# daiszh/A-TVSNet

Hardware: AMD Instinct MI355X
Metric: depth-maps/sec at 640x512xD=192, N=5 views (higher is better)
Workload: dtype f32 (fp16x2 split operands); 1 GPU; 1 depth map(s) per step: 5 views (1 ref + 4 src) 640x512, D=192, example.py multi-view pipeline; voxels=3932160, parallelism=single GPU, world_size=1, rccl_ranks=0, launch=HIP graph replay, batched per-view networks, inflight=1

## Files before the change

### a-tvsnet_amd/csrc/conv_stem.hip

```cpp
#include "conv_common.h"

namespace {

constexpr int ST_TZ = 4, ST_TY = 8, ST_TX = 32;
constexpr int ST_HZ = ST_TZ + 2, ST_HY = ST_TY + 2, ST_HX = ST_TX + 2;
typedef unsigned u32x4 __attribute__((ext_vector_type(4)));
__device__ float rs_zeros[8];
constexpr int RS_PF = (ST_HZ * ST_HY * ST_HX + 255) / 256;
#ifndef RS_WAVES
#define RS_WAVES 2
#endif
constexpr int RS_GRID = RS_WAVES * 256;
constexpr int RS_STG = 64 * 9;

template <int CIN>
__global__ __launch_bounds__(256) void conv_stem_kernel(const float* __restrict__ x, const float* __restrict__ w,
                                                        const float* __restrict__ pbias, float* __restrict__ y,
                                                        double* __restrict__ stats, int D, int H, int W, int ldy, int ycoff,
                                                        int relu, int tiles_y, int tiles_x, int tiles) {
  __shared__ float tile[ST_HZ * ST_HY * ST_HX * CIN];
  __shared__ double s_red[4][2][8];
  const int tid = threadIdx.x;
  const int grp = blockIdx.x / tiles, t = blockIdx.x - grp * tiles;
  const int x0 = (t % tiles_x) * ST_TX, y0 = ((t / tiles_x) % tiles_y) * ST_TY, z0 = (t / (tiles_x * tiles_y)) * ST_TZ;
  const size_t vol = (size_t)D * H * W;
  const float* xg = x + (size_t)grp * vol * CIN;
  for (int s = tid; s < ST_HZ * ST_HY * ST_HX * CIN; s += 256) {
    const int c = s % CIN, v = s / CIN;
    const int xx = v % ST_HX, yy = (v / ST_HX) % ST_HY, zz = v / (ST_HX * ST_HY);
    const int gz = z0 + zz - 1, gy = y0 + yy - 1, gx = x0 + xx - 1;
    float val = 0.f;
    if ((unsigned)gz < (unsigned)D && (unsigned)gy < (unsigned)H && (unsigned)gx < (unsigned)W)
      val = xg[(((size_t)gz * H + gy) * W + gx) * CIN + c];
    tile[s] = val;
  }
  __syncthreads();
  const int lx = tid & 31, ly = tid >> 5;
  const int xo = x0 + lx, yo = y0 + ly;
  const bool col_ok = xo < W && yo < H;
  float acc[ST_TZ][8];
#pragma unroll
  for (int z = 0; z < ST_TZ; ++z)
#pragma unroll
    for (int k = 0; k < 8; ++k) acc[z][k] = 0.f;
#pragma unroll 1
  for (int kd = 0; kd < 3; ++kd)
#pragma unroll 1
    for (int j = 0; j < 9; ++j) {
      const float* wk = w + ((kd * 9 + j) * CIN) * 8;
      float wr[CIN][8];
#pragma unroll
      for (int c = 0; c < CIN; ++c)
#pragma unroll
// ... 222 lines not shown
        const bool ok = yy < H && xx < W && zo < D;
        const u32x4 bits = {__builtin_bit_cast(unsigned, v.x), __builtin_bit_cast(unsigned, v.y),
                            __builtin_bit_cast(unsigned, v.z), __builtin_bit_cast(unsigned, v.w)};
        const unsigned off = ok ? (unsigned)(((z * H + yy) * W + xx) * 8 + hf * 4) * 4u : ybytes;
        __builtin_amdgcn_raw_buffer_store_b128(bits, c == 0 ? yrsrc : (c == 1 ? yrsrc1 : yrsrc2), off, 0, ATVS_BUF_NT);
      }
    } else
#pragma unroll
    for (int i = 0; i < 8; ++i) {
      const int r = i >> 2, xi = (i & 3) * 8 + (lane >> 3), c = lane & 7;
      const float4 v = stg[(r * 32 + xi) * 9 + c];
      const int yy = y0 + 2 * wave + r, xx = x0 + xi;
      const bool ok = yy < H && xx < W && zo < D;
      const u32x4 bits = {__builtin_bit_cast(unsigned, v.x), __builtin_bit_cast(unsigned, v.y),
                          __builtin_bit_cast(unsigned, v.z), __builtin_bit_cast(unsigned, v.w)};
      __builtin_amdgcn_raw_buffer_store_b128(bits, yrsrc, ok ? (unsigned)(((z * H + yy) * W + xx) * 32 + c * 4) * 4u : ybytes, 0, ATVS_BUF_NT);
    }
    __builtin_amdgcn_fence(__ATOMIC_RELEASE, "wavefront");
    __builtin_amdgcn_wave_barrier();
    __builtin_amdgcn_fence(__ATOMIC_ACQUIRE, "wavefront");
  }
  if (stats) {
    double v[48];
#pragma unroll
    for (int k = 0; k < 24; ++k) {
      v[k] = (double)ssum[k];
      v[24 + k] = (double)ssq[k];
    }
    int c0 = 0;
    rs_halve<24>(v, 1, lane, c0);
    rs_halve<12>(v, 2, lane, c0);
    rs_halve<6>(v, 4, lane, c0);
    rs_halve<3>(v, 8, lane, c0);
#pragma unroll
    for (int i = 0; i < 3; ++i) {
      v[i] += __shfl_xor(v[i], 16);
      v[i] += __shfl_xor(v[i], 32);
    }
    if (lane < 16) {
      double* row = &s_red[wave][0][0];
#pragma unroll
      for (int i = 0; i < 3; ++i) row[c0 + i] = v[i];
    }
    __syncthreads();
    if (tid < 48) {
      const int which = tid / 24, col = tid % 24;
      stats[((size_t)id * 2 + which) * 24 + col] =
          (s_red[0][which][col] + s_red[1][which][col]) + (s_red[2][which][col] + s_red[3][which][col]);
    }
  }
  }
}

}

extern "C" long atvs_conv_stem_rows(int D, int H, int W) {
  return (long)((D + ST_TZ - 1) / ST_TZ) * ((H + ST_TY - 1) / ST_TY) * ((W + ST_TX - 1) / ST_TX);
}

extern "C" int atvs_conv_stem_f32(const float* x, const float* w, const float* plane_bias, float* y, double* stats_partial,
                                  int groups, int D, int H, int W, int Cin, int ldy, int y_coff, int relu,
                                  atvs_stream_t stream) {
  if (!x || !w || !y) return ATVS_ERR_NULL;
  if (groups <= 0 || D <= 0 || H <= 0 || W <= 0 || (Cin != 1 && Cin != 2)) return ATVS_ERR_SHAPE;
  if (y_coff < 0 || y_coff + 8 > ldy || (ldy % 4) || (y_coff % 4)) return ATVS_ERR_SHAPE;
  if (plane_bias && D < 2) return ATVS_ERR_ARG;
  const int ty = (H + ST_TY - 1) / ST_TY, tx = (W + ST_TX - 1) / ST_TX;
  const long tiles = atvs_conv_stem_rows(D, H, W);
  if (tiles * groups > 0x7fffffffL) return ATVS_ERR_SHAPE;
  dim3 grid((unsigned)(tiles * groups)), block(256);
  hipStream_t s = as_stream(stream);
  if (Cin == 1)
    hipLaunchKernelGGL((conv_stem_kernel<1>), grid, block, 0, s, x, w, plane_bias, y, stats_partial, D, H, W, ldy, y_coff, relu,
                       ty, tx, (int)tiles);
  else
    hipLaunchKernelGGL((conv_stem_kernel<2>), grid, block, 0, s, x, w, plane_bias, y, stats_partial, D, H, W, ldy, y_coff, relu,
                       ty, tx, (int)tiles);
  ATVS_LAUNCH_CHECK();
  return ATVS_OK;
}

extern "C" int atvs_refine_stems_f32(const float* photo_raw, const float* geo, const float* geo_plane_bias, const float* prob,
                                     const float* hull, const float* w, float* y, double* stats_partial, int groups, int D,
                                     int H, int W, long y_planar, atvs_stream_t stream) {
  if ((!photo_raw && !y_planar) || !geo || !prob || !hull || !w || !y) return ATVS_ERR_NULL;
  if (groups <= 0 || D <= 0 || H <= 0 || W <= 0) return ATVS_ERR_SHAPE;
  if (y_planar && y_planar < (long)D * H * W * 8) return ATVS_ERR_ARG;
  if (geo_plane_bias && D < 2) return ATVS_ERR_ARG;
  if ((double)H * W * 128.0 * ST_TZ >= 4294967296.0) return ATVS_ERR_SHAPE;
  const int ty = (H + ST_TY - 1) / ST_TY, tx = (W + ST_TX - 1) / ST_TX;
  const long tiles = atvs_conv_stem_rows(D, H, W);
  if (tiles * groups > 0x7fffffffL) return ATVS_ERR_SHAPE;
  const long total = tiles * groups;
  const dim3 grid((unsigned)(total < RS_GRID ? total : RS_GRID));
  if (y_planar)
    hipLaunchKernelGGL(refine_stems_kernel<true>, grid, dim3(256), 0, as_stream(stream), photo_raw, geo, geo_plane_bias, prob,
                       hull, w, y, stats_partial, D, H, W, ty, tx, (int)tiles, groups, y_planar);
  else
    hipLaunchKernelGGL(refine_stems_kernel<false>, grid, dim3(256), 0, as_stream(stream), photo_raw, geo, geo_plane_bias, prob,
                       hull, w, y, stats_partial, D, H, W, ty, tx, (int)tiles, groups, 0L);
  ATVS_LAUNCH_CHECK();
  return ATVS_OK;
}

extern "C" int atvs_refine_stems_pack(const float* w_geo, const float* w_prob, const float* w_hull, float* packed) {
  if (!w_geo || !w_prob || !w_hull || !packed) return ATVS_ERR_NULL;
  for (int t = 0; t < 27; ++t)
    for (int k = 0; k < 8; ++k) {
      packed[(t * 4 + 0) * 8 + k] = w_geo[(t * 2 + 0) * 8 + k];
      packed[(t * 4 + 1) * 8 + k] = w_geo[(t * 2 + 1) * 8 + k];
      packed[(t * 4 + 2) * 8 + k] = w_prob[t * 8 + k];
      packed[(t * 4 + 3) * 8 + k] = w_hull[t * 8 + k];
    }
  return ATVS_OK;
}
```

### a-tvsnet_amd/ops/base.py

```python

import ctypes
import os

import torch

from .. import _lib


_ERR = {-1: 'null pointer', -2: 'bad shape', -3: 'bad argument', -4: 'launch failed'}


class Config(object):
    _DEFAULTS = dict(
        split16=os.environ.get('ATVS_SPLIT16', '1') == '1',
        split_off=frozenset(v for v in os.environ.get('ATVS_SPLIT_OFF', '').split(',') if v),
        xb=os.environ.get('ATVS_SPLIT16', '1') == '1',
        planar=True,
        pieces=os.environ.get('ATVS_PIECES', '1') == '1',
        planar_concat=os.environ.get('ATVS_PLANAR_CONCAT', '1') != '0',
        conv_c16=True, deconv_up=True, stem=True, conv2d_lds=True, conv1x1=True, xp1w=True, xpair=True, siblings=True,
        aanet_fused=os.environ.get('ATVS_AANET_FUSED', '1') != '0',
        bottleneck=os.environ.get('ATVS_BOTTLENECK', '1') != '0',
        prologue=True, sum_on_load=os.environ.get('ATVS_SUM_ON_LOAD', '1') != '0',
        norm3d=os.environ.get('ATVS_NORM3D', '1') != '0', head_sum=os.environ.get('ATVS_HEAD_SUM', '1') != '0',
        force_impl=None, fused_finalize=False,
        side_streams=os.environ.get('ATVS_SIDE_STREAMS', '1') != '0')

    def __init__(self):
        for k, v in self._DEFAULTS.items():
            object.__setattr__(self, k, v)

    def __setattr__(self, name, value):
        if name not in self._DEFAULTS:
            raise AttributeError('ops.cfg has no switch %r (known: %s)' % (name, ', '.join(sorted(self._DEFAULTS))))
        if name == 'split_off':
            value = frozenset(value)
        elif name == 'force_impl':
            if value not in (None, 'tiled', 'gather'):
                raise ValueError('force_impl: None | "tiled" | "gather"')
        else:
            value = bool(value)
        object.__setattr__(self, name, value)
        if name == 'split16':
            object.__setattr__(self, 'xb', value)

    def snapshot(self):
        return {k: getattr(self, k) for k in self._DEFAULTS}


cfg = Config()


class configure(object):

    def __init__(self, clear_pack_cache=False, **switches):
        for k in switches:
            if k not in Config._DEFAULTS:
                raise AttributeError('ops.cfg has no switch %r' % k)
        self._new, self._clear = switches, clear_pack_cache

    def __enter__(self):
        self._old = cfg.snapshot()
        for k in sorted(self._new, key=lambda n: n != 'split16'):
            setattr(cfg, k, self._new[k])
        if self._clear:
            from .packing import clear_pack_cache
            clear_pack_cache()
        return cfg

    def __exit__(self, *exc):
        for k, v in self._old.items():
            object.__setattr__(cfg, k, v)
        if self._clear:
            from .packing import clear_pack_cache
            clear_pack_cache()
        return False

# ... 123 lines not shown
```

### a-tvsnet_amd/ops/convolution.py

```python

import ctypes

import torch

from .. import _lib
from .base import _Timed, _call, _dev_ok, _new, _p, _side_stream, _stats, _stats_buffer, _stream, cfg
from .packing import (_abi_pack, _fold_cache, _virt_cache, _xkind, conv_taps, deconv_s2_class_taps, deconv_up_ok,
    pack_conv3d_b, pack_conv_c16, pack_conv_c16b, pack_conv_weights, pack_conv_weights_tiled, pack_conv_xp,
    pack_conv_xp_sibling, pack_deconv_up, planar_pieces_decode, planar_stride, planar_view, split_on)
from .geometry import tile_planes
from .norm import LAZY, PendingBN, PendingSum, _param_groups, bn_apply, channel_stats, copy_channels, siblings_prologue_ok
from .launch import (Fin, XPAIR_TAPS, _fin_counter, _from5, _to5, _xpair_virtual_kernel, conv1x1, conv2d_lds, conv_blocks,
    conv_launch, conv_plan, conv_tiled_launch, conv_xp_launch, pack_conv2d_lds, tiled_blocks, tiled_tile_y, xp_blocks)


def conv(x, key, w_host, stride=1, dilation=1, padding='SAME', explicit_pad=None, bias=None, residual=None,
         relu=False, want_stats=False, out=None, y_coff=0, plane_bias=None, groups=None, in_params=None,
         in_relu=False, in_sum=None):
    x5, nsp = _to5(x, groups, 'conv input')
    G, ins = x5.shape[0], tuple(x5.shape[1:4])
    cin, cout = int(w_host.shape[-2]), int(w_host.shape[-1])
    if cin != x5.shape[4]:
        raise ValueError('conv %s: input has %d channels, kernel wants %d' % (key, x5.shape[4], cin))
    y5 = _to5(out, groups, 'conv output buffer')[0] if out is not None else None
# ... 224 lines not shown
    cv, cc = sv.cv, sv.const.shape[-1]
    wv, planes = _fold_split_weights(key, w_host, sv.chan_map, cv, cc)
    pb = conv(sv.const, (key, 'planes'), planes, stride=stride, groups=B)
    return conv(sv.var, (key, 'var'), wv, stride=stride, want_stats=want_stats, plane_bias=pb, out=out, y_coff=y_coff,
                groups=B)


def planar_concat_ok(shape):
    D, h, w = (int(v) for v in shape)
    return (cfg.planar_concat and cfg.planar and _xkind() == 'xb' and cfg.prologue and cfg.force_impl is None
            and siblings_ok((D, h, w), 32, 8, 16) and 4.0 * 4 * planar_stride(D, h, w) < 2.0 ** 40)


def photo_pieces_ok(shape, chan):
    return cfg.pieces and chan in (16, 32, 64) and planar_concat_ok(shape)


def conv_split_into_plane(sv, key, w_host, buf, plane, planar):
    D, H, W = planar
    B, K, pstride = buf.shape
    if (sv.planar and (not sv.pieces or sv.planar != (D, H, W))) or sv.shape[0] != B or tuple(sv.shape[1:4]) != (D, H, W) or pstride != planar_stride(D, H, W) \
            or not buf.is_contiguous() or int(w_host.shape[-1]) != 8 or sv.cv % 8:
        raise ValueError('conv_split_into_plane: shapes')
    cv, cc = sv.cv, sv.const.shape[-1]
    wv, planes = _fold_split_weights(key, w_host, sv.chan_map, cv, cc)
    pb = conv(sv.const, (key, 'planes'), planes, stride=1, groups=B)
    pk = pack_conv_xp((key, 'var'), wv, buf.device)
    if pk.kind != 'xb':
        raise ValueError('conv_split_into_plane: the split-fp16 x-pair kernel only')
    blocks = xp_blocks(D, H, W, B)
    st, sbuf = _stats(buf, blocks, 16, D * H * W, B)
    if sv.pieces:
        conv_xp_launch(sv._var, pk, buf, 0, None, False, sbuf, pb, ldy=8, y_gstride=K * pstride, y_off=int(plane) * pstride,
                       planar=sv.planar, pieces=True)
    else:
        conv_xp_launch(sv.var, pk, buf, 0, None, False, sbuf, pb, ldy=8, y_gstride=K * pstride, y_off=int(plane) * pstride)
    return st


def refine_stems(photo_raw, geo_var, geo_plane_bias, prob, hull, key, w_geo, w_prob, w_hull, planar_out=None):
    import numpy as np
    B, D, H, W, _ = geo_var.shape
    if planar_out is not None and (tuple(planar_out.shape) != (B, 4, planar_stride(D, H, W)) or not planar_out.is_contiguous()):
        raise ValueError('refine_stems: planar_out must be a contiguous (B, 4, planar_stride(D,h,w)) buffer')
    photo_raw = geo_var if planar_out is not None else photo_raw
    if tuple(np.shape(w_geo)) != (3, 3, 3, 2, 8) or tuple(np.shape(w_prob)) != (3, 3, 3, 1, 8) \
            or tuple(np.shape(w_hull)) != (3, 3, 3, 1, 8):
        raise ValueError('refine_stems: kernels [3,3,3,2,8], [3,3,3,1,8], [3,3,3,1,8]')
    pk = _abi_pack('stems', key, (w_geo, w_prob, w_hull), photo_raw.device, 'refine_stems_pack', 27 * 4 * 8, cin=4, cout=24)
    buf = _new(photo_raw, (B, D, H, W, 32)) if planar_out is None else planar_out
    st, sbuf = _stats(photo_raw, _lib.lib().atvs_conv_stem_rows(D, H, W), 24, D * H * W, B)
    if _dev_ok(photo_raw, geo_var, geo_plane_bias, prob, hull, buf):
        with _Timed(key, (D, H, W, 4), 24, B):
            _call('atvs_refine_stems_f32', _p(photo_raw if planar_out is None else None), _p(geo_var), _p(geo_plane_bias),
                  _p(prob), _p(hull), _p(pk.wp), _p(buf), _p(sbuf), B, D, H, W,
                  ctypes.c_long(planar_stride(D, H, W) if planar_out is not None else 0), _stream())
    return buf, st


def siblings_ok(shape, cin, cout, cout2):
    return (cfg.xp1w and cfg.xpair and cfg.siblings and cfg.force_impl != 'gather' and len(shape) == 3 and cout == 8
            and cout2 == 16 and cin % 8 == 0 and (shape[2] >= 24 or cfg.force_impl == 'tiled'))


def conv_siblings(x, key, w_host, key2, w2_host, plane_bias=None, plane_bias2=None, groups=None, planar=False, pieces=False):
    prologue = None
    if isinstance(x, LAZY):
        if not siblings_prologue_ok(x):
            raise ValueError('conv_siblings: this lazy input must be materialised first')
        if isinstance(x, PendingBN) and x.planar and x._final is None:
            planar = x.planar
        x, prologue = x.prologue()
    if planar:
        D, H, W = planar
        if (prologue is not None and _xkind() != 'xb') or groups is None or x.dim() != 3 \
                or not x.is_contiguous() or x.shape[2] != planar_stride(D, H, W):
            raise ValueError('conv_siblings(planar=(D,H,W)): a contiguous (G, Cin/8, planar_stride) buffer (a prologue only '
                             'on the split-fp16 kernel)')
        G, K = x.shape[:2]
        x5, nsp, cin = x, 3, K * 8
    else:
        x5, nsp = _to5(x, groups, 'conv_siblings input')
        G, D, H, W, cin = x5.shape
    if nsp != 3 or not siblings_ok((D, H, W), cin, int(w_host.shape[-1]), int(w2_host.shape[-1])):
        raise ValueError('conv_siblings: unsupported shapes')
    pk = pack_conv_xp(key, w_host, x.device)
    pk2 = pack_conv_xp_sibling(key2, w2_host, x.device)
    if pk.cin != cin or pk2.cin != cin:
        raise ValueError('conv_siblings %s: input has %d channels' % (key, cin))
    D2, H2, W2 = (D + 1) // 2, (H + 1) // 2, (W + 1) // 2
    lead = () if groups is None else (G,)
    y, y2 = _new(x, lead + (D, H, W, 8)), _new(x, lead + (D2, H2, W2, 16))
    blocks = xp_blocks(D, H, W, G)
    st, sbuf = _stats(x, blocks, 16, D * H * W, G)
    st2, sbuf2 = _stats(x, blocks, 16, D2 * H2 * W2, G)
    if plane_bias is not None and tuple(plane_bias.shape) != lead + (H, W, 24):
        raise ValueError('conv_siblings %s: plane_bias %s' % (key, tuple(plane_bias.shape)))
    if plane_bias2 is not None and tuple(plane_bias2.shape) != lead + (H2, W2, 48):
        raise ValueError('conv_siblings %s: plane_bias2 %s' % (key2, tuple(plane_bias2.shape)))
    if prologue is not None and prologue[0] is not None:
        prologue = (_to5(prologue[0], groups, 'conv_siblings second source')[0],) + tuple(prologue[1:])
    if pieces and (not planar or prologue is not None or _xkind() != 'xb'):
        raise ValueError('conv_siblings(pieces=True): a chunk-planar input without a prologue, on the split-operand kernel')
    conv_xp_launch(x5, pk, y, 0, None, False, sbuf, plane_bias, sibling=(pk2, y2, 0, sbuf2, plane_bias2),
                   prologue=prologue, planar=planar, pieces=pieces)
    return (y, st), (y2, st2)

# ... 177 lines not shown
```

### include/atvsnet_hip.h

```cpp
#ifndef ATVSNET_HIP_H
#define ATVSNET_HIP_H

#include <stddef.h>
#include <stdint.h>

#ifdef __cplusplus
extern "C" {
#endif

typedef void* atvs_stream_t;

enum {
  ATVS_OK = 0,
  ATVS_ERR_NULL = -1,
  ATVS_ERR_SHAPE = -2,
  ATVS_ERR_ARG = -3,
  ATVS_ERR_LAUNCH = -4
};

#define ATVS_ABI_VERSION 50
int atvs_abi_version(void);
const char* atvs_target_arch(void);


int atvs_get_homographies(const float* left_cam, const float* right_cam, const float* depth_start,
                          const float* depth_interval, float* homographies, int depth_num,
                          int inverse_depth, atvs_stream_t stream);

int atvs_warp_planes(const float* src, const float* homographies, const float* ref,
                     const float* depth_start, const float* depth_interval, float* out, float* mask_out,
                     int D, int h, int w, int C, int ld_out, int c_off, int mode, int rep, long planar, int pieces,
                     atvs_stream_t stream);

int atvs_build_cost_volume(const float* ref_feature, const float* view_feature, const float* homographies,
                           float* cost_volume, int D, int h, int w, int C, atvs_stream_t stream);

int atvs_tile_planes(const float* src, float* out, int D, int h, int w, int C, int ld_out, int c_off,
                     atvs_stream_t stream);

int atvs_geo_ref_planes(const float* depth_ref, const float* depth_start, const float* depth_interval,
                        float* out, int D, int h, int w, int ld_out, int c_off, atvs_stream_t stream);
int atvs_geo_volume(const float* depth_ref, const float* view_depth, const float* homographies, const float* depth_start,
                    const float* depth_interval, float* out, int D, int h, int w, int ld_out, int c_off, int rep,
                    atvs_stream_t stream);

int atvs_visual_hull(const float* ref_depth, const float* view_depth_in_ref, const float* homographies,
                     const float* depth_start, const float* depth_interval, float* out, int D, int h, int w,
                     int inverse_depth, atvs_stream_t stream);

int atvs_warp_by_depth(const float* src, const float* left_cam, const float* right_cam, const float* depth,
                       float* out, float* mask_out, float* pose_ws, int h, int w, int C, int method,
                       int inverse_depth, atvs_stream_t stream);

int atvs_warp_by_depth_err(const float* src, const float* ref, const float* left_cam, const float* right_cam,
                           const float* depth, float* out, int ld_out, int c_off, int h, int w, int C, int method,
                           int inverse_depth, int copy_ref, atvs_stream_t stream);

int atvs_interpolate(const float* src, const float* x, const float* y, float* out, float* mask_out, long n,
                     int h, int w, int C, int method, atvs_stream_t stream);

int atvs_pixel_grids(float* out, int h, int w, atvs_stream_t stream);

int atvs_transform_depth(const float* depth, const float* left_cam, const float* right_cam, float* out,
                         float* ws14, int h, int w, int inverse_depth, atvs_stream_t stream);
int atvs_transform_depth_batch_supported(int h, int w);
int atvs_transform_depth_batch(const float* const* depth, const float* const* left_cam, const float* const* right_cam,
                               float* const* out, int n, int h, int w, int inverse_depth, atvs_stream_t stream);

int atvs_absdiff_mask(const float* a, const float* b, const float* mask, float* out, int npix, int C,
                      atvs_stream_t stream);


int atvs_softargmin(const float* cost, const float* depth_start, const float* depth_interval,
// ... 95 lines not shown
int atvs_conv1x1_b_pack_size(int Cin, int Cout, long* packed_bytes);
int atvs_conv1x1_b_pack(const float* w, int Cin, int Cout, unsigned char* packed);
long atvs_conv1x1_b_rows(long pixels);
int atvs_conv1x1_b_f32(const float* x, const unsigned char* packed_w, const float* bias, const float* residual,
                       const float* in_params, int in_relu, float* y, double* stats_partial, int groups, long pixels,
                       int Cin, int Cout, int ldy, int y_coff, int relu, atvs_stream_t stream);

int atvs_bottleneck_b_supported(int C, int dilation);
long atvs_bottleneck_b_rows(int C, int H, int W);
int atvs_bottleneck_b_f32(const float* x, const float* in_params, const unsigned char* w1, const float* b1,
                          const unsigned char* w2, const float* b2, const unsigned char* w3, const float* b3, float* y,
                          double* stats_partial, int G, int H, int W, int C, int dilation, atvs_stream_t stream);

int atvs_conv3d_b_supported(int Cin, int Cout);
int atvs_conv3d_b_pack_size(int Cin, int Cout, long* packed_bytes);
int atvs_conv3d_b_pack(const float* w, int Cin, int Cout, unsigned char* packed);
int atvs_conv3d_b_f32(const float* x, const unsigned char* packed_w, const float* bias, float* y, double* stats_partial,
                      int groups, int D, int H, int W, int Cin, int Cout, int ldy, int y_coff, int relu, atvs_stream_t stream);
int atvs_conv3d_b_norm_f32(const float* x, const float* in_params, int in_relu, const unsigned char* packed_w, const float* bias,
                           float* y, double* stats_partial, int groups, int D, int H, int W, int Cin, int Cout, int ldy,
                           int y_coff, int relu, atvs_stream_t stream);

int atvs_conv3d_s2b_supported(int Cin, int Cout);
long atvs_conv3d_s2b_grid(int Do, int Ho, int Wo, int groups);
int atvs_conv3d_s2b_pack_size(int Cin, int Cout, long* packed_bytes);
int atvs_conv3d_s2b_pack(const float* w, int Cin, int Cout, unsigned char* packed);
int atvs_conv3d_s2b_f32(const float* x, const unsigned char* packed_w, const float* bias, float* y, double* stats_partial,
                        int groups, int D, int H, int W, int Cin, int Cout, int ldy, int y_coff, int relu, atvs_stream_t stream);
int atvs_conv3d_s2b_norm_f32(const float* x, const float* in_params, int in_relu, const unsigned char* packed_w,
                             const float* bias, float* y, double* stats_partial, int groups, int D, int H, int W, int Cin,
                             int Cout, int ldy, int y_coff, int relu, atvs_stream_t stream);

long atvs_deconv_up_b_grid(int D, int H, int W, int Cout, int groups);
int atvs_deconv_up_b_supported(int Cin, int Cout);
int atvs_deconv_up_b_pack_size(int Cin, int Cout, long* packed_bytes);
int atvs_deconv_up_b_pack(const float* w, int Cin, int Cout, unsigned char* packed);
int atvs_deconv_up_b_f32(const float* x, const unsigned char* packed_w, float* y, double* stats_partial, int groups, int D, int H,
                         int W, int Cin, int Cout, int ldy, int y_coff, int relu, int stats_ld, int stats_coff,
                         atvs_stream_t stream);

int atvs_deconv_up_b_sum_supported(int Cin, int Cout);
int atvs_deconv_up_b_sum_f32(const float* x0, const float* params0, const float* x1, const float* params1, const float* x2,
                             const float* params2, int relu_mask, const unsigned char* packed_w, float* y, double* stats_partial,
                             int groups, int D, int H, int W, int Cin, int Cout, int ldy, int y_coff, int relu, int stats_ld,
                             int stats_coff, atvs_stream_t stream);
long atvs_conv_stem_rows(int D, int H, int W);
int atvs_conv_stem_f32(const float* x, const float* w, const float* plane_bias, float* y, double* stats_partial,
                       int groups, int D, int H, int W, int Cin, int ldy, int y_coff, int relu, atvs_stream_t stream);

int atvs_refine_stems_pack(const float* w_geo, const float* w_prob, const float* w_hull, float* packed);
int atvs_refine_stems_f32(const float* photo_raw, const float* geo, const float* geo_plane_bias, const float* prob,
                          const float* hull, const float* w, float* y, double* stats_partial, int groups, int D, int H,
                          int W, long y_planar, atvs_stream_t stream);

int atvs_conv3d_8to1(const float* x, const float* w, float* y, int groups, int D, int H, int W, atvs_stream_t stream);
int atvs_conv3d_8to1_bn2(const float* x0, const float* params0, const float* x1, const float* params1, int relu_mask,
                         const float* w, float* y, int groups, int D, int H, int W, atvs_stream_t stream);



int atvs_bn_finalize(const double* stats_partial, int groups, long num_blocks, int cpad, int fold, long count,
                     const float* beta, float eps, float* params, int C, int* nonfinite_flag, atvs_stream_t stream);

long atvs_channel_stats_num_blocks(long rows);
int atvs_channel_stats(const float* x, int groups, long rows, int C, double* stats_partial, atvs_stream_t stream);

int atvs_bn_apply(const float* x, const float* params, float* y, int groups, long rows, int C, int ld, int c_off,
                  int relu, atvs_stream_t stream);

int atvs_bn_add(const float* x0, const float* params0, const float* x1, const float* params1, const float* x2,
                const float* params2, float* y, int groups, long rows, int C, int relu_mask, atvs_stream_t stream);
int atvs_bn_add_plus(const float* x0, const float* params0, const float* x1, const float* params1, const float* x2,
                     const float* params2, float* y, const float* base, float* y2, int groups, long rows, int C, int relu_mask,
                     atvs_stream_t stream);

int atvs_add_n(const float* a, const float* b, const float* c, float* y, long n, atvs_stream_t stream);

long atvs_avg_pool_ws_floats(int H, int W, int C, int stride);
int atvs_avg_pool_same(const float* x, float* y, float* ws, int groups, int H, int W, int C, int pool, int stride,
                       atvs_stream_t stream);

int atvs_resize_bilinear(const float* x, float* y, int groups, int H, int W, int C, int Ho, int Wo, int ld_out,
                         int c_off, atvs_stream_t stream);

int atvs_copy_channels(const float* src, float* dst, long rows, int C, int ld_src, int src_off, int ld_dst,
                       int dst_off, atvs_stream_t stream);

int atvs_stack(const float* const* srcs, int n, long elems, float* dst, atvs_stream_t stream);


int atvs_aanet_combine(const float* const* sr_ptrs, const float* const* x_ptrs, int nv, float* out, long V,
                       atvs_stream_t stream);

int atvs_aanet_b_supported(int C, int nv);
int atvs_aanet_b_pack_size(long* packed_bytes);
int atvs_aanet_b_pack(const float* w_shared, const float* w_unique, unsigned char* packed);
int atvs_aanet_b_f32(const float* const* x, int nv, const unsigned char* packed_w, float* out, int D, int H, int W,
                     atvs_stream_t stream);

int atvs_aanet_partial(const float* const* sr_ptrs, const float* const* x_ptrs, int nv, int stage,
                       const float* ssum, const float* umax, float* out, long V, atvs_stream_t stream);

int atvs_divide(const float* num, const float* den, float* out, long n, atvs_stream_t stream);


int atvs_fusibile(const float* cams, const float* normals_depths, const float* images, int nviews, int ref, int rows,
// ... 80 lines not shown
```

Before: 59.90 depth-maps/sec.

## Split refine-stems kernel into producer/consumer wave roles with double-buffered halo

Adds a 512-thread persistent refine_stems kernel with specialized wavefronts. Four waves run the 27-tap FMA loop from LDS with software-pipelined weight and voxel loads. The other four waves, at raised priority, prefetch the next tile's halo into a second LDS buffer through buffer loads and handle bias, statistics and output stores. The aim is to overlap global memory latency and epilogue work with the tap arithmetic that the previous single-role kernel ran serially. In exchange it uses a large dynamic LDS footprint, one block per CU, and extra LDS barriers. An env switch, on by default, keeps the old kernel selectable.

Result: no change. 60.31 depth-maps/sec, median of 3 (+0.7%).

```diff
diff --git a/a-tvsnet_amd/csrc/conv_stem.hip b/a-tvsnet_amd/csrc/conv_stem.hip
--- a/a-tvsnet_amd/csrc/conv_stem.hip
+++ b/a-tvsnet_amd/csrc/conv_stem.hip
@@ -1,4 +1,10 @@
 #include "conv_common.h"
+
+typedef float rs_f32x2 __attribute__((ext_vector_type(2)));
+__device__ rs_f32x2 rs_buffer_load_x2(__amdgpu_buffer_rsrc_t rsrc, int voffset, int soffset, int aux)
+    __asm("llvm.amdgcn.raw.ptr.buffer.load.v2f32");
+__device__ float rs_buffer_load_x1(__amdgpu_buffer_rsrc_t rsrc, int voffset, int soffset, int aux)
+    __asm("llvm.amdgcn.raw.ptr.buffer.load.f32");
 
 namespace {
 
@@ -327,6 +333,332 @@
   }
 }
 
+constexpr int RS_IMG = ST_HZ * ST_HY * ST_HX;
+constexpr int RS2_SLOT = 4 * RS_STG;
+constexpr int RS2_LDS = (2 * RS_IMG + 2 * RS2_SLOT) * 16 + 4 * 48 * 8;
+constexpr int RS2_GRID = 256;
+
+#ifdef ATVS_RS_DEBUG
+__device__ unsigned long long atvs_dbg_rs[256 * 8 * 8];
+#define RSDBG(i) { unsigned long long t_ = clock64(); dbg_acc[i] += t_ - dbg_t; dbg_t = t_; }
+#else
+#define RSDBG(i)
+#endif
+
+struct RsTaps { int b[32]; };
+constexpr RsTaps rs_make_taps() {
+  RsTaps t{};
+  for (int i = 0; i < 27; ++i) t.b[i] = (((i / 9) * ST_HY + (i % 9) / 3) * ST_HX + i % 3) * 16;
+  return t;
+}
+__constant__ RsTaps rs_taps = rs_make_taps();
+
+__device__ __forceinline__ void rs_lds_barrier() { asm volatile("s_waitcnt lgkmcnt(0)\n\ts_barrier" ::: "memory"); }
+
+template <bool PLANAR>
+__global__ __launch_bounds__(512, 1) void refine_stems_kernel_roles(const float* __restrict__ photo, const float* __restrict__ geo,
+                                                                  const float* __restrict__ geo_pb, const float* __restrict__ prob,
+                                                                  const float* __restrict__ hull, const float* __restrict__ w,
+                                                                  float* __restrict__ y, double* __restrict__ stats, int D, int H,
+                                                                  int W, int tiles_y, int tiles_x, int tiles, int groups, long pstride) {
+  extern __shared__ __attribute__((aligned(16))) unsigned char rs_smem[];
+  float4* const img = reinterpret_cast<float4*>(rs_smem);
+  float4* const slots = img + 2 * RS_IMG;
+  double* const s_red = reinterpret_cast<double*>(slots + 2 * RS2_SLOT);
+  const int tid = threadIdx.x & 255, lane = tid & 63;
+  const int wave = __builtin_amdgcn_readfirstlane(threadIdx.x >> 6), w4 = wave & 3;
+  const size_t vol = (size_t)D * H * W;
+  const int total = tiles * groups;
+  const int n = (total - (int)blockIdx.x + (int)gridDim.x - 1) / (int)gridDim.x;
+#ifdef ATVS_RS_DEBUG
+  unsigned long long dbg_acc[8] = {0, 0, 0, 0, 0, 0, 0, 0};
+  unsigned long long dbg_t = clock64();
+#endif
+
+  if (wave < 4) {
+    typedef float f32x2 __attribute__((ext_vector_type(2)));
+    const int lx = tid & 31, ly = tid >> 5;
+    rs_lds_barrier();
+#pragma unroll 1
+    for (int i = 0; i < n; ++i) {
+      const float4* im = img + (i & 1) * RS_IMG + ly * ST_HX + lx;
+      f32x2 acc2[ST_TZ][12];
+#pragma unroll
+      for (int z = 0; z < ST_TZ; ++z)
+#pragma unroll
+        for (int k = 0; k < 12; ++k) acc2[z][k] = (f32x2){0.f, 0.f};
+      typedef const float __attribute__((address_space(4))) * rs_cptr;
+      uintptr_t wa_ = reinterpret_cast<uintptr_t>(w);
+      asm volatile("" : "+s"(wa_));
+      const rs_cptr wt = reinterpret_cast<rs_cptr>(wa_);
+      f32x4 v0[ST_TZ], v1[ST_TZ];
+      f32x2 wA[8], wB[8];
+      int ob1 = rs_taps.b[1], ob2 = rs_taps.b[2];
+      auto issue_v = [&](int tp, f32x4* vb, int ob) __attribute__((always_inline)) {
+        const f32x4* src = reinterpret_cast<const f32x4*>(reinterpret_cast<const unsigned char*>(im) + ob);
+#pragma unroll
+        for (int z = 0; z < ST_TZ; ++z) vb[z] = src[z * ST_HY * ST_HX];
+      };
+      auto issue_w = [&](int tp, int part, f32x2* wb) __attribute__((always_inline)) {
+        const rs_cptr wk = wt + tp * 32 + part * 16;
+#pragma unroll
+        for (int k = 0; k < 8; ++k) wb[k] = (f32x2){wk[2 * k], wk[2 * k + 1]};
+      };
+      auto pin = [&](f32x4* vb) __attribute__((always_inline)) {
+#pragma unroll
+        for (int z = 0; z < ST_TZ; ++z) asm volatile("" : "+v"(vb[z]));
+      };
+      auto tap = [&](int tp, f32x4* vc, f32x4* vn, int ob, bool more) __attribute__((always_inline)) {
+        pin(vc);
+#pragma unroll
+        for (int z = 0; z < ST_TZ; ++z) {
+          const f32x2 vx = {vc[z].x, vc[z].x}, vy = {vc[z].y, vc[z].y};
+#pragma unroll
+          for (int k = 0; k < 4; ++k) {
+            acc2[z][k] = __builtin_elementwise_fma(vx, wA[k], acc2[z][k]);
+            acc2[z][k] = __builtin_elementwise_fma(vy, wA[4 + k], acc2[z][k]);
+          }
+        }
+        __builtin_amdgcn_sched_barrier(0);
+        __builtin_amdgcn_s_waitcnt(0xc07f);
+        if (more) {
+          issue_w(tp + 1, 0, wA);
+          issue_v(tp + 1, vn, ob);
+        }
+        __builtin_amdgcn_sched_barrier(0);
+#pragma unroll
+        for (int z = 0; z < ST_TZ; ++z) {
+          const f32x2 vz = {vc[z].z, vc[z].z}, vw = {vc[z].w, vc[z].w};
+#pragma unroll
+          for (int k = 0; k < 4; ++k) {
+            acc2[z][4 + k] = __builtin_elementwise_fma(vz, wB[k], acc2[z][4 + k]);
+            acc2[z][8 + k] = __builtin_elementwise_fma(vw, wB[4 + k], acc2[z][8 + k]);
+          }
+        }
+        __builtin_amdgcn_sched_barrier(0);
+        __builtin_amdgcn_s_waitcnt(0xc07f);
+        if (more) issue_w(tp + 1, 1, wB);
+        __builtin_amdgcn_sched_barrier(0);
+      };
+      issue_w(0, 0, wA);
+      issue_w(0, 1, wB);
+      issue_v(0, v0, 0);
+      __builtin_amdgcn_s_waitcnt(0xc07f);
+#pragma unroll 1
+      for (int tp = 0; tp < 26; tp += 2) {
+        const int nb1 = rs_taps.b[tp + 3], nb2 = rs_taps.b[tp + 4];
+        tap(tp, v0, v1, ob1, true);
+        tap(tp + 1, v1, v0, ob2, true);
+        ob1 = nb1;
+        ob2 = nb2;
+      }
+      tap(26, v0, v1, 0, false);
+      RSDBG(0)
+#pragma unroll
+      for (int z = 0; z < ST_TZ; ++z) {
+        float4* stg = slots + (z & 1) * RS2_SLOT + w4 * RS_STG;
+#pragma unroll
+        for (int k = 0; k < 12; k += 2) stg[lane * 9 + 2 + k / 2] = make_float4(acc2[z][k].x, acc2[z][k].y, acc2[z][k + 1].x, acc2[z][k + 1].y);
+        RSDBG(1)
+        rs_lds_barrier();
+        RSDBG(2)
+      }
+    }
+    rs_lds_barrier();
+#ifdef ATVS_RS_DEBUG
+    if (lane == 0) {
+      dbg_acc[7] = (unsigned long long)n;
+      for (int j = 0; j < 8; ++j) atvs_dbg_rs[(blockIdx.x * 8 + wave) * 8 + j] = dbg_acc[j];
+    }
+#endif
+    return;
+  }
+
+#ifndef ATVS_RS_PRIO
+#define ATVS_RS_PRIO 3
+#endif
+  __builtin_amdgcn_s_setprio(ATVS_RS_PRIO);
+  float4 pf[RS_PF];
+  int rel[RS_PF], hyy[RS_PF], hxx[RS_PF];
+#pragma unroll
+  for (int i = 0; i < RS_PF; ++i) {
+    const int s = tid + i * 256;
+    const int xx = s % ST_HX, yy = (s / ST_HX) % ST_HY, zz = s / (ST_HX * ST_HY);
+    rel[i] = (zz * H + yy) * W + xx;
+    hyy[i] = s < RS_IMG ? yy : -0x40000000;
+    hxx[i] = xx;
+  }
+  auto request = [&](int id) __attribute__((always_inline)) {
+    const int grp = id / tiles, t = id - grp * tiles;
+    const int x0 = (t % tiles_x) * ST_TX, y0 = ((t / tiles_x) % tiles_y) * ST_TY, z0 = (t / (tiles_x * tiles_y)) * ST_TZ;
+    const unsigned vbytes = (unsigned)vol * 4u;
+    const __amdgpu_buffer_rsrc_t grs = __builtin_amdgcn_make_buffer_rsrc(const_cast<float*>(geo) + (size_t)grp * vol * 2, 0, 2 * vbytes, 0x00020000);
+    const __amdgpu_buffer_rsrc_t prs = __builtin_amdgcn_make_buffer_rsrc(const_cast<float*>(prob) + (size_t)grp * vol, 0, vbytes, 0x00020000);
+    const __amdgpu_buffer_rsrc_t hrs = __builtin_amdgcn_make_buffer_rsrc(const_cast<float*>(hull) + (size_t)grp * vol, 0, vbytes, 0x00020000);
+    const int vb = ((z0 - 1) * H + (y0 - 1)) * W + (x0 - 1);
+    const int ylo = 1 - y0, xlo = 1 - x0;
+#pragma unroll
+    for (int i = 0; i < RS_PF; ++i) {
+      const int vx = vb + rel[i];
+      const bool ok = (unsigned)(hyy[i] - ylo) < (unsigned)H && (unsigned)(hxx[i] - xlo) < (unsigned)W && vx >= 0;
+      const int o4 = ok ? vx * 4 : 0x40000000;
+      const rs_f32x2 g2 = rs_buffer_load_x2(grs, o4 * 2, 0, 0);
+      pf[i] = make_float4(g2.x, g2.y, rs_buffer_load_x1(prs, o4, 0, 0), rs_buffer_load_x1(hrs, o4, 0, 0));
+    }
+  };
+  auto land = [&](float4* image) __attribute__((always_inline)) {
+#pragma unroll
+    for (int i = 0; i < RS_PF; ++i)
+      if (tid + i * 256 < RS_IMG) image[tid + i * 256] = pf[i];
+  };
+  auto stats_row = [&](int id) __attribute__((always_inline)) {
+    typedef unsigned u32x2 __attribute__((ext_vector_type(2)));
+    const int c = tid < 48 ? tid : 47;
+    const double s4 = (s_red[c] + s_red[48 + c]) + (s_red[96 + c] + s_red[144 + c]);
+    const __amdgpu_buffer_rsrc_t srsrc = __builtin_amdgcn_make_buffer_rsrc(stats + (size_t)id * 48, 0, 384, 0x00020000);
+    __builtin_amdgcn_raw_buffer_store_b64(__builtin_bit_cast(u32x2, s4), srsrc, tid < 48 ? (unsigned)tid * 8u : 384u, 0, 0);
+  };
+  request(blockIdx.x);
+  land(img);
+  request(n > 1 ? blockIdx.x + gridDim.x : blockIdx.x);
+  rs_lds_barrier();
+  const int lx = tid & 31, ly = tid >> 5;
+#pragma unroll 1
+  for (int i = 0; i < n; ++i) {
+    const int id = blockIdx.x + i * gridDim.x;
+    const int grp = id / tiles, t = id - grp * tiles;
+    const int x0 = (t % tiles_x) * ST_TX, y0 = ((t / tiles_x) % tiles_y) * ST_TY, z0 = (t / (tiles_x * tiles_y)) * ST_TZ;
+    land(img + ((i + 1) & 1) * RS_IMG);
+    RSDBG(0)
+    request(blockIdx.x + (i + 2 < n ? i + 2 : n - 1) * gridDim.x);
+    float* yg = PLANAR ? y + (size_t)grp * 4 * pstride + pstride : y + (size_t)grp * vol * 32;
+    const unsigned ybytes = (unsigned)((size_t)H * W * (PLANAR ? 32 : 128) * ST_TZ);
+    const __amdgpu_buffer_rsrc_t yrsrc = __builtin_amdgcn_make_buffer_rsrc(yg + (size_t)z0 * H * W * (PLANAR ? 8 : 32), 0, ybytes, 0x00020000);
+    const __amdgpu_buffer_rsrc_t yrsrc1 = __builtin_amdgcn_make_buffer_rsrc(yg + (PLANAR ? pstride : 0) + (size_t)z0 * H * W * 8, 0, ybytes, 0x00020000);
+    const __amdgpu_buffer_rsrc_t yrsrc2 = __builtin_amdgcn_make_buffer_rsrc(yg + (PLANAR ? 2 * pstride : 0) + (size_t)z0 * H * W * 8, 0, ybytes, 0x00020000);
+    const int xo = x0 + lx, yo = y0 + ly;
+    const bool col_ok = xo < W && yo < H;
+    const float* pbg = geo_pb ? geo_pb + (size_t)grp * H * W * 24 : nullptr;
+    float4 bb[ST_TZ][2];
+#pragma unroll
+    for (int z = 0; z < ST_TZ; ++z) {
+      const bool ok = col_ok && z0 + z < D;
+      const float* pb = ok && pbg ? pbg + ((size_t)yo * W + xo) * 24 + plane_variant(z0 + z - 1, D) * 8 : rs_zeros;
+      bb[z][0] = ld4(pb);
+      bb[z][1] = ld4(pb + 4);
+    }
+    float ssum[24], ssq[24];
+#pragma unroll
+    for (int k = 0; k < 24; ++k) ssum[k] = ssq[k] = 0.f;
+    float4 ph[ST_TZ][2];
+    if (!PLANAR) {
+      const float* phg = photo + (size_t)grp * vol * 8;
+#pragma unroll
+      for (int z = 0; z < ST_TZ; ++z) {
+        const bool ok = xo < W && yo < H && z0 + z < D;
+        const float* pp = ok ? phg + (((size_t)(z0 + z) * H + yo) * W + xo) * 8 : rs_zeros;
+        ph[z][0] = ld4(pp);
+        ph[z][1] = ld4(pp + 4);
+      }
+    }
+    RSDBG(1)
+#pragma unroll
+    for (int z = 0; z < ST_TZ; ++z) {
+      const int zo = z0 + z;
+      rs_lds_barrier();
+      RSDBG(2)
+      float4* stg = slots + (z & 1) * RS2_SLOT + w4 * RS_STG;
+      if (z == 0 && i > 0 && stats) stats_row(id - (int)gridDim.x);
+      {
+        float a24[24];
+#pragma unroll
+        for (int k = 0; k < 24; k += 4) {
+          const float4 q = stg[lane * 9 + 2 + k / 4];
+          a24[k] = q.x; a24[k + 1] = q.y; a24[k + 2] = q.z; a24[k + 3] = q.w;
+        }
+        const float4 b0 = bb[z][0], b1 = bb[z][1];
+        if (pbg) {
+          a24[0] += b0.x; a24[1] += b0.y; a24[2] += b0.z; a24[3] += b0.w;
+          a24[4] += b1.x; a24[5] += b1.y; a24[6] += b1.z; a24[7] += b1.w;
+          stg[lane * 9 + 2] = make_float4(a24[0], a24[1], a24[2], a24[3]);
+          stg[lane * 9 + 3] = make_float4(a24[4], a24[5], a24[6], a24[7]);
+        }
+        const bool ok = col_ok && zo < D;
+#pragma unroll
+        for (int k = 0; k < 24; ++k) {
+          const float a = ok ? a24[k] : 0.f;
+          ssum[k] += a;
+          ssq[k] += a * a;
+        }
+      }
+      if (!PLANAR) {
+        stg[lane * 9] = ph[z][0];
+        stg[lane * 9 + 1] = ph[z][1];
+      }
+      __builtin_amdgcn_fence(__ATOMIC_RELEASE, "wavefront");
+      __builtin_amdgcn_wave_barrier();
+      __builtin_amdgcn_fence(__ATOMIC_ACQUIRE, "wavefront");
+      if (PLANAR) {
+#pragma unroll
+        for (int j = 0; j < 6; ++j) {
+          const int c = j >> 1, r = j & 1, xi = lane >> 1, hf = lane & 1;
+          const float4 q = stg[(r * 32 + xi) * 9 + 2 + c * 2 + hf];
+          const int yy = y0 + 2 * w4 + r, xx = x0 + xi;
+          const bool ok = yy < H && xx < W && zo < D;
+          const u32x4 bits = {__builtin_bit_cast(unsigned, q.x), __builtin_bit_cast(unsigned, q.y),
+                              __builtin_bit_cast(unsigned, q.z), __builtin_bit_cast(unsigned, q.w)};
+          const unsigned off = ok ? (unsigned)(((z * H + yy) * W + xx) * 8 + hf * 4) * 4u : ybytes;
+          __builtin_amdgcn_raw_buffer_store_b128(bits, c == 0 ? yrsrc : (c == 1 ? yrsrc1 : yrsrc2), off, 0, ATVS_BUF_NT);
+        }
+      } else {
+#pragma unroll
+        for (int j = 0; j < 8; ++j) {
+          const int r = j >> 2, xi = (j & 3) * 8 + (lane >> 3), c = lane & 7;
+          const float4 q = stg[(r * 32 + xi) * 9 + c];
+          const int yy = y0 + 2 * w4 + r, xx = x0 + xi;
+          const bool ok = yy < H && xx < W && zo < D;
+          const u32x4 bits = {__builtin_bit_cast(unsigned, q.x), __builtin_bit_cast(unsigned, q.y),
+                              __builtin_bit_cast(unsigned, q.z), __builtin_bit_cast(unsigned, q.w)};
+          __builtin_amdgcn_raw_buffer_store_b128(bits, yrsrc, ok ? (unsigned)(((z * H + yy) * W + xx) * 32 + c * 4) * 4u : ybytes, 0, ATVS_BUF_NT);
+        }
+      }
+      RSDBG(3)
+    }
+    if (stats) {
+      double sv[48];
+#pragma unroll
+      for (int k = 0; k < 24; ++k) {
+        sv[k] = (double)ssum[k];
+        sv[24 + k] = (double)ssq[k];
+      }
+      int c0 = 0;
+      rs_halve<24>(sv, 1, lane, c0);
+      rs_halve<12>(sv, 2, lane, c0);
+      rs_halve<6>(sv, 4, lane, c0);
+      rs_halve<3>(sv, 8, lane, c0);
+#pragma unroll
+      for (int j = 0; j < 3; ++j) {
+        sv[j] += __shfl_xor(sv[j], 16);
+        sv[j] += __shfl_xor(sv[j], 32);
+      }
+      if (lane < 16) {
+        double* row = s_red + w4 * 48;
+#pragma unroll
+        for (int j = 0; j < 3; ++j) row[c0 + j] = sv[j];
+      }
+    }
+    RSDBG(4)
+  }
+  rs_lds_barrier();
+  if (stats) stats_row((int)blockIdx.x + (n - 1) * (int)gridDim.x);
+#ifdef ATVS_RS_DEBUG
+  if (lane == 0) {
+    dbg_acc[7] = (unsigned long long)n;
+    for (int j = 0; j < 8; ++j) atvs_dbg_rs[(blockIdx.x * 8 + wave) * 8 + j] = dbg_acc[j];
+  }
+#endif
+}
+
 }
 
 extern "C" long atvs_conv_stem_rows(int D, int H, int W) {
@@ -355,9 +687,9 @@
   return ATVS_OK;
 }
 
-extern "C" int atvs_refine_stems_f32(const float* photo_raw, const float* geo, const float* geo_plane_bias, const float* prob,
-                                     const float* hull, const float* w, float* y, double* stats_partial, int groups, int D,
-                                     int H, int W, long y_planar, atvs_stream_t stream) {
+static int refine_stems_launch(bool roles, const float* photo_raw, const float* geo, const float* geo_plane_bias, const float* prob,
+                               const float* hull, const float* w, float* y, double* stats_partial, int groups, int D, int H, int W,
+                               long y_planar, atvs_stream_t stream) {
   if ((!photo_raw && !y_planar) || !geo || !prob || !hull || !w || !y) return ATVS_ERR_NULL;
   if (groups <= 0 || D <= 0 || H <= 0 || W <= 0) return ATVS_ERR_SHAPE;
   if (y_planar && y_planar < (long)D * H * W * 8) return ATVS_ERR_ARG;
@@ -367,6 +699,21 @@
   const long tiles = atvs_conv_stem_rows(D, H, W);
   if (tiles * groups > 0x7fffffffL) return ATVS_ERR_SHAPE;
   const long total = tiles * groups;
+  if (roles && (double)D * H * W < 134217728.0) {
+    const dim3 grid((unsigned)(total < RS2_GRID ? total : RS2_GRID));
+    static AtvsAttrOnce once_planar, once_rows;
+    if (y_planar) {
+      if (const int rc_ = atvs_set_max_lds_once(once_planar, reinterpret_cast<const void*>(&refine_stems_kernel_roles<true>), RS2_LDS)) return rc_;
+      hipLaunchKernelGGL(refine_stems_kernel_roles<true>, grid, dim3(512), RS2_LDS, as_stream(stream), photo_raw, geo, geo_plane_bias,
+                         prob, hull, w, y, stats_partial, D, H, W, ty, tx, (int)tiles, groups, y_planar);
+    } else {
+      if (const int rc_ = atvs_set_max_lds_once(once_rows, reinterpret_cast<const void*>(&refine_stems_kernel_roles<false>), RS2_LDS)) return rc_;
+      hipLaunchKernelGGL(refine_stems_kernel_roles<false>, grid, dim3(512), RS2_LDS, as_stream(stream), photo_raw, geo, geo_plane_bias,
+                         prob, hull, w, y, stats_partial, D, H, W, ty, tx, (int)tiles, groups, 0L);
+    }
+    ATVS_LAUNCH_CHECK();
+    return ATVS_OK;
+  }
   const dim3 grid((unsigned)(total < RS_GRID ? total : RS_GRID));
   if (y_planar)
     hipLaunchKernelGGL(refine_stems_kernel<true>, grid, dim3(256), 0, as_stream(stream), photo_raw, geo, geo_plane_bias, prob,
@@ -378,6 +725,24 @@
   return ATVS_OK;
 }
 
+extern "C" int atvs_refine_stems_f32(const float* photo_raw, const float* geo, const float* geo_plane_bias, const float* prob,
+                                     const float* hull, const float* w, float* y, double* stats_partial, int groups, int D,
+                                     int H, int W, long y_planar, atvs_stream_t stream) {
+  return refine_stems_launch(true, photo_raw, geo, geo_plane_bias, prob, hull, w, y, stats_partial, groups, D, H, W, y_planar, stream);
+}
+
+extern "C" int atvs_refine_stems_serial_f32(const float* photo_raw, const float* geo, const float* geo_plane_bias, const float* prob,
+                                            const float* hull, const float* w, float* y, double* stats_partial, int groups, int D,
+                                            int H, int W, long y_planar, atvs_stream_t stream) {
+  return refine_stems_launch(false, photo_raw, geo, geo_plane_bias, prob, hull, w, y, stats_partial, groups, D, H, W, y_planar, stream);
+}
+
+#ifdef ATVS_RS_DEBUG
+extern "C" int atvs_debug_read_rs(void* host) {
+  return (int)hipMemcpyFromSymbol(host, HIP_SYMBOL(atvs_dbg_rs), sizeof(atvs_dbg_rs));
+}
+#endif
+
 extern "C" int atvs_refine_stems_pack(const float* w_geo, const float* w_prob, const float* w_hull, float* packed) {
   if (!w_geo || !w_prob || !w_hull || !packed) return ATVS_ERR_NULL;
   for (int t = 0; t < 27; ++t)
diff --git a/a-tvsnet_amd/ops/base.py b/a-tvsnet_amd/ops/base.py
--- a/a-tvsnet_amd/ops/base.py
+++ b/a-tvsnet_amd/ops/base.py
@@ -23,6 +23,7 @@
         bottleneck=os.environ.get('ATVS_BOTTLENECK', '1') != '0',
         prologue=True, sum_on_load=os.environ.get('ATVS_SUM_ON_LOAD', '1') != '0',
         norm3d=os.environ.get('ATVS_NORM3D', '1') != '0', head_sum=os.environ.get('ATVS_HEAD_SUM', '1') != '0',
+        stems_roles=os.environ.get('ATVS_STEMS_ROLES', '1') != '0',
         force_impl=None, fused_finalize=False,
         side_streams=os.environ.get('ATVS_SIDE_STREAMS', '1') != '0')
 
diff --git a/a-tvsnet_amd/ops/convolution.py b/a-tvsnet_amd/ops/convolution.py
--- a/a-tvsnet_amd/ops/convolution.py
+++ b/a-tvsnet_amd/ops/convolution.py
@@ -300,7 +300,8 @@
     st, sbuf = _stats(photo_raw, _lib.lib().atvs_conv_stem_rows(D, H, W), 24, D * H * W, B)
     if _dev_ok(photo_raw, geo_var, geo_plane_bias, prob, hull, buf):
         with _Timed(key, (D, H, W, 4), 24, B):
-            _call('atvs_refine_stems_f32', _p(photo_raw if planar_out is None else None), _p(geo_var), _p(geo_plane_bias),
+            _call('atvs_refine_stems_f32' if cfg.stems_roles else 'atvs_refine_stems_serial_f32',
+                  _p(photo_raw if planar_out is None else None), _p(geo_var), _p(geo_plane_bias),
                   _p(prob), _p(hull), _p(pk.wp), _p(buf), _p(sbuf), B, D, H, W,
                   ctypes.c_long(planar_stride(D, H, W) if planar_out is not None else 0), _stream())
     return buf, st
diff --git a/include/atvsnet_hip.h b/include/atvsnet_hip.h
--- a/include/atvsnet_hip.h
+++ b/include/atvsnet_hip.h
@@ -18,7 +18,7 @@
   ATVS_ERR_LAUNCH = -4
 };
 
-#define ATVS_ABI_VERSION 50
+#define ATVS_ABI_VERSION 51
 int atvs_abi_version(void);
 const char* atvs_target_arch(void);
 
@@ -220,6 +220,9 @@
 int atvs_refine_stems_f32(const float* photo_raw, const float* geo, const float* geo_plane_bias, const float* prob,
                           const float* hull, const float* w, float* y, double* stats_partial, int groups, int D, int H,
                           int W, long y_planar, atvs_stream_t stream);
+int atvs_refine_stems_serial_f32(const float* photo_raw, const float* geo, const float* geo_plane_bias, const float* prob,
+                                 const float* hull, const float* w, float* y, double* stats_partial, int groups, int D, int H,
+                                 int W, long y_planar, atvs_stream_t stream);
 
 int atvs_conv3d_8to1(const float* x, const float* w, float* y, int groups, int D, int H, int W, atvs_stream_t stream);
 int atvs_conv3d_8to1_bn2(const float* x0, const float* params0, const float* x1, const float* params1, int relu_mask,
diff --git a/tools_dev/phase_rs.py b/tools_dev/phase_rs.py
--- /dev/null
+++ b/tools_dev/phase_rs.py
@@ -0,0 +1,28 @@
+import sys, os, ctypes
+sys.path.insert(0, os.path.dirname(os.path.dirname(os.path.abspath(__file__))))
+import numpy as np
+import torch
+import atvsnet_amd
+from atvsnet_amd import ops, _lib
+dev = torch.device('cuda:0')
+torch.manual_seed(0)
+G, D, H, W = 4, 192, 128, 160
+geo, prob, hull = (torch.randn(G, D, H, W, c, device=dev) for c in (2, 1, 1))
+pb = torch.randn(G, H, W, 24, device=dev)
+ws = [(torch.randn(3, 3, 3, c, 8) * 0.1).numpy() for c in (2, 1, 1)]
+buf = torch.zeros(G, 4, ops.planar_stride(D, H, W), device=dev)
+for _ in range(3):
+    ops.refine_stems(None, geo, pb, prob, hull, 'phase-rs', *ws, planar_out=buf)
+torch.cuda.synchronize()
+raw = np.zeros(256 * 8 * 8, np.uint64)
+assert _lib.lib().atvs_debug_read_rs(raw.ctypes.data_as(ctypes.c_void_p)) == 0
+t = raw.reshape(256, 8, 8).astype(np.float64)
+ns = t[:, 0, 7].mean()
+for role, sl, names in (('computing wavefronts', slice(0, 4), ['taps', 'slot writes', 'barriers']),
+                        ('memory wavefronts', slice(4, 8), ['wait for the halo + land', 'next halo + bias requests', 'barriers (the taps)',
+                                                            'planes: bias, statistics, stores', 'butterfly + statistics row'])):
+    r = t[:, sl, :].reshape(-1, 8)
+    tot = r[:, :len(names)].sum(1).mean()
+    print('%s: %.1f stages each, %.0f ticks per stage' % (role, ns, tot / ns))
+    for i, n in enumerate(names):
+        print('   %-42s %8.0f per stage (%.1f%%)' % (n, r[:, i].mean() / ns, 100 * r[:, i].mean() / tot))
```
